# BioinformaticsToolsmith/MeShClust

Hardware: AMD Instinct MI355X
Metric: sequences clustered/sec (+ NW cell-updates/sec) at 1/2/4/8 MI355X (higher is better)
Workload: dtype u8

## Files before the change

meshclust_amd/csrc/gpu/accum_impl.hpp:

```cpp
#pragma once
#include <algorithm>
#include <cstdlib>
#include <cstring>

#include "bvec_core.hpp"
#include "features.hpp"

namespace mcg {

namespace {

constexpr int NT = 512;
constexpr int NW = NT / 64;
constexpr uint32_t NONE = 0xffffffffu;
constexpr uint64_t NONE64 = ~0ull;
constexpr uint32_t RING = 64;
constexpr uint32_t TRACE_STEPS = 4096;
constexpr int TRACE_W = 20;
constexpr uint32_t TRACE2_STEPS = 256;
constexpr int T2W = 6;
constexpr int KINL = 4;
constexpr int REC_HDR = 14;
constexpr uint32_t REC_EXACT = 0x80000000u, REC_THIN = 0x40000000u, REC_KMASK = 0x3fffffffu;
constexpr int PART_G = 8;
// ... 53 lines not shown
  int etake;
  int xfast;
  int thin;
  int rpoll;
  int rpoll_gap;
  uint32_t rec_g;
  uint64_t *klog;
  uint32_t *go;
  uint64_t *partials;
  uint32_t *fpos;
  uint64_t fcap;
  int res;
  uint4 *cc;
  uint4 *srows;
  uint32_t dres;
  uint32_t mrow;
  uint32_t *mem_pos;
  uint64_t *mkeys;
  uint32_t *cl_centre;
  uint64_t *cl_off;
  uint64_t *out;
  uint64_t budget;
  int prof;
  uint64_t *trace;
  int trace_all;
  uint64_t *trace2;
  uint32_t W, rank;
  uint64_t *mbox;
  uint64_t slot_g;
};

__device__ __forceinline__ uint64_t now() { return __builtin_amdgcn_s_memrealtime(); }

typedef unsigned int u32x4_t __attribute__((ext_vector_type(4)));
__device__ __forceinline__ uint4 ld_nt16(const uint4 *p) {
  const u32x4_t v = __builtin_nontemporal_load(reinterpret_cast<const u32x4_t *>(p));
  return make_uint4(v.x, v.y, v.z, v.w);
}

#define MC_LDS __attribute__((address_space(3)))
#define MC_GLB __attribute__((address_space(1)))
__device__ __forceinline__ uint32_t lds_u32(const uint32_t *p) { return *(const MC_LDS uint32_t *)p; }
__device__ __forceinline__ uint64_t lds_u64(const uint64_t *p) { return *(const MC_LDS uint64_t *)p; }
__device__ __forceinline__ uint4 lds_u4(const uint4 *p) {
  const u32x4_t v = *(const MC_LDS u32x4_t *)p;
  return make_uint4(v.x, v.y, v.z, v.w);
}
__device__ __forceinline__ void glb_st16(MC_GLB u32x4_t *p, const uint4 &v) { *p = (u32x4_t){v.x, v.y, v.z, v.w}; }
__device__ __forceinline__ void lds_st16(MC_LDS u32x4_t *p, const uint4 &v) { *p = (u32x4_t){v.x, v.y, v.z, v.w}; }
__device__ __forceinline__ uint4 lds_ld16(const MC_LDS u32x4_t *p) {
  const u32x4_t v = *p;
  return make_uint4(v.x, v.y, v.z, v.w);
}
__device__ __forceinline__ WinTab lds_wt(const WinTab *p) {
  static_assert(sizeof(WinTab) == 40, "WinTab is read as five 8-byte words");
  const MC_LDS uint64_t *q = (const MC_LDS uint64_t *)p;
  uint64_t w[5];
#pragma unroll
  for (int i = 0; i < 5; i++) w[i] = q[i];
  WinTab r;
  __builtin_memcpy(&r, w, sizeof(WinTab));
  return r;
}

__device__ __forceinline__ void trace_mark(const AccArgs &A, uint32_t step, int slot, uint64_t t) {
  if (!A.trace || !A.trace_all || step >= TRACE_STEPS) return;
// ... 508 lines not shown
            uint4 v[NC];
#pragma unroll
            for (int k = 0; k < NC; k++)
              v[k] = from_hs ? A.hs[(uint64_t)k * A.npad + pos] : ld_nt16(creg + (uint64_t)k * NT + t);
            const PInfo pi{A.mag_s[pos], A.sumsq_s[pos], A.len_s[pos]};
            Acc<T> acc;
            double cv;
#pragma unroll
            for (int k = 0; k < NC; k++) acc.add(v[k], clds[k]);
            if (classify_cand<T>(acc, pi, pc, A.B, C, &cv)) {
              lal[(uint64_t)li * NT + sl] = 0;
              flag_pos(pos);
            }
            if (cv > -1.0 && better(cv, pos, best_v, best_p)) {
              best_v = cv;
              best_p = pos;
            }
          }
        }
      }
    } else
    for (uint64_t ch = c0 + mine; ch <= c1; ch += GW) {
      const uint64_t li = dgw.div((uint32_t)ch);
      const uint64_t pos = (ch * A.W + A.rank) * NT + threadIdx.x;
      uint8_t *la = lal + li * NT + threadIdx.x;
      if (!(pos >= P_S && pos <= P_E && *la)) continue;
      nscan++;
      if (trace && threadIdx.x == 0) t_top = now();
      Acc<T> acc;
      double cv;
      if ((int64_t)li < res) {
        const uint4 *rr = lrow + li * (uint64_t)nch * NT + threadIdx.x;
        if constexpr (NCH > 0) {
          constexpr int HB = NC >= 8 ? 8 : NC;
#pragma unroll
          for (int k0 = 0; k0 < NC; k0 += HB) {
            uint4 rv[HB], cvv[HB];
#pragma unroll
            for (int k = 0; k < HB; k++) {
              rv[k] = rr[(uint64_t)(k0 + k) * NT];
              cvv[k] = clds[k0 + k];
            }
#pragma unroll
            for (int k = 0; k < HB; k++) acc.add(rv[k], cvv[k]);
          }
        } else {
          for (int k = 0; k < nch; k++) acc.add(rr[(uint64_t)k * NT], clds[k]);
        }
        if constexpr (sizeof(T) == 1)
          if (trace && threadIdx.x == 0) {
            acc.fold();
            asm volatile("" ::"v"(acc.sad), "v"(acc.dot));
            t_sad = now();
          }
        int d;
        if (li < 2 && C.layout) {
          const PInfo pi = li == 0 ? rinf0 : rinf1;
          d = classify_std(C, acc.finish(pi.mag, pc.mag), pi, li == 0 ? rterm0 : rterm1, pc, tq, A.B, &cv);
#ifdef MC_EXP_DOUBLE_CLASSIFY
          {
            double cv2;
            PInfo p2 = pi;
            const uint64_t z = (uint64_t)(A.budget >> 62);
            p2.len += z;
            p2.mag += z;
            p2.sumsq += z;
            const int d2 = classify_std(C, acc.finish(p2.mag, pc.mag), p2, pterms(p2.mag, p2.sumsq, A.B), pc, tq, A.B, &cv2);
// ... 276 lines not shown
    const PTerms tq = pterms_mk(pc.mag, pc.sumsq, A.B, A.fc.rB);
    const PSm ps_q = psmall(pc, tq);
    const double kq = (double)((int64_t)pc.mag - (int64_t)A.B * tq.ap);
    {
      const uint32_t kinl0 = kend > (uint32_t)KINL ? kend - KINL : 0;
      const uint64_t t0k = kinl0 > kcur ? now() : 0;
      for (uint32_t e = kcur; e < kend; e++) {
        uint32_t p;
        if (e >= kinl0) {
          p = hdr[4 + KINL - (kend - e)];
        } else {
          uint64_t g = ld64(A.klog + e);
          for (uint32_t it = 1; (uint32_t)(g >> 32) != e + 1; it++) {
            if ((it & 255) == 0 && timed_out(A, t0k)) {
              s_abort = 1;
              break;
            }
            __builtin_amdgcn_s_sleep(1);
            g = ld64(A.klog + e);
          }
          p = (uint32_t)g;
        }
        if (p == pos_t) al_t = false;
      }
      kcur = kend;
    }
    if (trace && t == 0) t_klog = now();
    const bool comp = al_t && pos_t >= P_S && pos_t <= P_E;
    int d_t = 0;
    double cv_t = -1.0;
    if (comp) {
      Acc<T> acc;
      const uint4 *rr = lrow + t;
      constexpr int HB = NC >= 8 ? 8 : NC;
      const SmallK sk = lds_smallk(&s_sk);
      if constexpr (NCH > 0) {
#pragma unroll
        for (int k0 = 0; k0 < NC; k0 += HB) {
          uint4 rv[HB], cvv[HB];
#pragma unroll
          for (int k = 0; k < HB; k++) {
            rv[k] = rr[(uint64_t)(k0 + k) * NT];
            cvv[k] = clds[k0 + k];
          }
#pragma unroll
          for (int k = 0; k < HB; k++) acc.add(rv[k], cvv[k]);
        }
      } else {
        for (int k = 0; k < nch; k++) acc.add(rr[(uint64_t)k * NT], clds[k]);
      }
      bool und = true;
      if constexpr (sizeof(T) == 1) {
        if (small_on && ps_q.ok && ps_t.ok) {
          acc.fold();
          d_t = classify_small(sk, acc.sad, acc.dot, ps_t, ps_q, kq, pt_t.da, tq.da, A.B, &cv_t, &und);
          if (und) {
            double cx;
            d_t = classify_std(C, acc.finish(pi_t.mag, pc.mag), pi_t, pt_t, pc, tq, A.B, &cx);
            und = false;
          }
        }
      }
      if (und)
        d_t = A.fc.on    ? classify_fast(C, A.fc, acc.finish(pi_t.mag, pc.mag), pi_t, pt_t, pc, tq, A.B, &cv_t)
              : C.layout ? classify_std(C, acc.finish(pi_t.mag, pc.mag), pi_t, pt_t, pc, tq, A.B, &cv_t)
                         : classify_cand<T>(acc, pi_t, pc, A.B, C, &cv_t);
    }
// ... 566 lines not shown
          }
          lpos[nxt][r] = lp[e];
        }
        base += tot;
        __syncthreads();
      }
      drain();
      __syncthreads();
      n_ent = base;
      alive = 0;
      for (uint32_t j = 0; j < J; j++)
        if (t + NT * j < n_ent) alive |= 1u << j;
      cur = nxt;
    }
  }
}

template <typename T, int NCH, bool WIDE, int TSZ, bool PROF>
__device__ __forceinline__ void controller(const AccArgs &A, uint4 *dyn) {
  [[maybe_unused]] const bool prof_on = PROF && A.prof;
  [[maybe_unused]] uint64_t *const trace = PROF ? A.trace : nullptr;
  [[maybe_unused]] uint64_t *const trace2 = PROF ? A.trace2 : nullptr;
  __shared__ uint64_t s_red[3 * NW];
  __shared__ double s_bv[NW];
  __shared__ uint64_t s_bp[NW];
  __shared__ uint32_t s_new;
  __shared__ uint32_t s_plist[PLIST];
  __shared__ uint32_t s_pbin[PLIST];
  __shared__ uint64_t s_q[4];
  __shared__ uint32_t s_klast[KINL];
  __shared__ uint32_t s_span_all;
  __shared__ int s_abort;
  __shared__ uint64_t s_sumF;
  __shared__ double s_xv[64];
  __shared__ uint64_t s_xp[64];
  __shared__ uint32_t s_xn[64], s_xs[64], s_xi[64][MBOX_INL];
  constexpr int NC = NCH > 0 ? NCH : 1;
  const uint32_t GW = gridDim.x - 1;
  const int lane = threadIdx.x & 63, wv = wave_id();
  const int nch = NCH > 0 ? NCH : A.nch;
  const int rec_words = (int)A.rec_g;
  uint8_t *Fl = reinterpret_cast<uint8_t *>(dyn);
  uint64_t *msum = reinterpret_cast<uint64_t *>(Fl + (size_t)nch * 16);
  uint32_t *cnt = reinterpret_cast<uint32_t *>(msum + A.B);
  uint32_t *fw = cnt + ((A.nb + 1) & ~1u);
  uint32_t *lo = fw + ((A.nb + 2) & ~1u);
  uint64_t *bnd = reinterpret_cast<uint64_t *>(lo + ((A.nb + 2) & ~1u));
  uint32_t *lbits = reinterpret_cast<uint32_t *>(bnd + A.nb);
  const uint64_t nwords = (A.N + 31) / 32;
  MemberCache mc;
  {
    uint8_t *p = reinterpret_cast<uint8_t *>(lbits + (A.gbits ? 0 : (nwords + 3) / 4 * 4));
    mc.rp = WIDE ? 0 : nch + 1;
    mc.row = reinterpret_cast<uint4 *>(p);
    p += (size_t)A.mrow * mc.rp * 16;
    mc.wt = reinterpret_cast<WinTab *>(p);
    p += (size_t)A.mrow * sizeof(WinTab);
    mc.info = reinterpret_cast<uint64_t *>(p);
    p += (size_t)A.mrow * 24;
    mc.key = reinterpret_cast<uint64_t *>(p);
    p += (size_t)A.mrow * 8;
    mc.pos = reinterpret_cast<uint32_t *>(p);
  }
  for (int i = threadIdx.x; i < nch * 16; i += NT) Fl[i] = 0;
  if (threadIdx.x == 0) {
    s_abort = 0;
    s_new = 0;
  }
  uint64_t lg = 1;
  while (lg * 2 <= A.nb) lg *= 2;
  const __amdgpu_buffer_rsrc_t prs =
      __builtin_amdgcn_make_buffer_rsrc(A.partials, 0, (int)(GW * PART_G * 8), 0x00020000);
  DevBvec bv{A.gbits, (MC_LDS uint32_t *)lbits, A.gbits != nullptr, cnt, fw, lo, bnd, A.len_s, A.nb, lg};
  uint32_t last = NONE;
  uint32_t last_q = 0;
  uint64_t cl_start = 0;
  uint64_t M = 0;
  uint64_t ncl = 0, nsteps = 0, ncand = 0;
  uint32_t step = 0;
  uint64_t err = 0;
  uint32_t kn = 0;
  bool rec_exact = false;
  bool thin_out = false;
  uint32_t npend = 0;
  uint64_t t_wait = 0, t_coll = 0, t_mark = 0;
  const uint64_t clk0 = prof_on ? __builtin_amdgcn_s_memtime() : 0, rt0 = prof_on ? now() : 0;
  uint64_t t_sub[4] = {0, 0, 0, 0};
  uint64_t t_ws[4] = {0, 0, 0, 0};
  uint64_t t_cl[3] = {0, 0, 0};
  uint64_t t_pub[2] = {0, 0};
  uint64_t t_wk[5] = {0, 0, 0, 0, 0};

  constexpr uint32_t BK = 64;
  auto finish_cluster = [&]() {
    if (threadIdx.x == BK) {
      A.cl_centre[ncl] = last;
      A.cl_off[ncl + 1] = cl_start + M;
    }
    ncl++;
    cl_start += M;
    M = 0;
  };
  auto log_kill = [&](uint64_t p) {
    if (threadIdx.x == BK) st64(A.klog + kn, gran(kn + 1, (uint32_t)p));
    if (threadIdx.x == 0) s_klast[kn % KINL] = (uint32_t)p;
  };
  auto new_cluster = [&](uint64_t pos, bool kill = false, bool logged = false) {
    if (A.mrow && !WIDE)
      for (int c = threadIdx.x; c < nch; c += NT) mc.row[c] = A.hr[pos * nch + c];
    for (int b = threadIdx.x; b < A.B; b += NT) msum[b] = reinterpret_cast<const T *>(A.hr + pos * nch)[b];
    if (kill && !logged) log_kill(pos);
    if (threadIdx.x == 0) {
      if (A.mrow) {
// ... 18 lines not shown
    M = 1;
    last_q = 0;
    if (kill && !logged) kn++;
    __syncthreads();
  };
  auto pop = [&]() -> uint64_t {
    const int64_t b = bv.first_nonempty();
    if (b < 0) return NONE64;
    const uint64_t p = bv.select((uint64_t)b, 0);
    if (threadIdx.x == 0) bv.kill_in(p, (uint64_t)b);
    log_kill(p);
    kn++;
    __syncthreads();
    return p;
  };
  auto rec_word = [&](int j, bool have, uint64_t S, uint64_t E) -> uint32_t {
    const bool cached = last_q < A.mrow;
    if (!WIDE && j < 4 * nch) {
      if (last == NONE) return 0;
      const uint4 v = cached ? lds_u4(mc.row + (size_t)last_q * mc.rp + j / 4) : A.hr[(uint64_t)last * nch + j / 4];
      return (j & 3) == 0 ? v.x : (j & 3) == 1 ? v.y : (j & 3) == 2 ? v.z : v.w;
    }
    const int h = j - (WIDE ? 0 : 4 * nch);
    if (h == 0) return have ? last : NONE;
    if (h == 1) return (uint32_t)S;
    if (h == 2) return (uint32_t)E;
    if (h == 3) return kn | (rec_exact ? 0x80000000u : 0u);
    if (h < 4 + KINL) {
      const int64_t e = (int64_t)kn - KINL + (h - 4);
      return e >= 0 ? s_klast[e % KINL] : NONE;
    }
    if (last == NONE) return 0;
    const int f = (h - 4 - KINL) / 2, hi = (h - 4 - KINL) & 1;
    const uint64_t v =
        cached ? lds_u64(mc.info + (size_t)last_q * 3 + f) : (f == 0 ? A.mag_s[last] : f == 1 ? A.sumsq_s[last] : A.len_s[last]);
    return hi ? (uint32_t)(v >> 32) : (uint32_t)v;
  };

  auto rec_word_cached = [&](int j, bool have, uint64_t S, uint64_t E) -> uint32_t {
    const int h = j - 4 * nch;
    const int64_t e = (int64_t)kn - KINL + (h - 4);
    const MC_LDS uint32_t *row = (const MC_LDS uint32_t *)(mc.row + (size_t)last_q * mc.rp);
    const MC_LDS uint32_t *inf = (const MC_LDS uint32_t *)(mc.info + (size_t)last_q * 3);
    const MC_LDS uint32_t *p = h < 0               ? row + j
                               : h < 4 + KINL      ? (const MC_LDS uint32_t *)s_klast + (e >= 0 ? (uint32_t)e % KINL : 0u)
                                                   : inf + (h - 4 - KINL);
    const uint32_t x = *p;
    if (h < 0) return x;
    if (h == 0) return have ? last : NONE;
    if (h == 1) return (uint32_t)S;
    if (h == 2) return (uint32_t)E;
    if (h == 3) return kn | (rec_exact ? 0x80000000u : 0u);
    if (h < 4 + KINL) return e >= 0 ? x : NONE;
    return x;
  };
  constexpr int PW = 4;
  auto rec_read = [&](int j0, uint64_t S, uint64_t E, bool have, uint32_t (&d)[PW]) {
    const bool fastw = !WIDE && last != NONE && last_q < A.mrow;
    if (fastw) {
#pragma unroll
      for (int u = 0; u < PW; u++) {
        const int j = j0 + u * 64 + lane;
        d[u] = j < rec_words ? rec_word_cached(j, have, S, E) : 0u;
      }
    } else {
#pragma unroll
      for (int u = 0; u < PW; u++) {
        const int j = j0 + u * 64 + lane;
// ... 5 lines not shown
    uint64_t *r = A.ring + (uint64_t)(step % RING) * A.rec_g;
#pragma unroll
    for (int u = 0; u < PW; u++) {
      const int j = j0 + u * 64 + lane;
      if (j < rec_words) st64(r + j, gran(step, d[u]));
    }
  };
  auto publish_thin = [&](uint32_t pos) {
    const int h = lane;
    const int64_t e = (int64_t)kn - KINL + (h - 4);
    const uint32_t kx = s_klast[e >= 0 ? (uint32_t)e % KINL : 0u];
    const uint32_t x = h == 0 ? pos : h == 1 ? 0u : h == 2 ? (uint32_t)(A.N - 1) : h == 3 ? (kn | REC_THIN)
                     : h < 4 + KINL ? (e >= 0 ? kx : NONE) : 0u;
    if (4 * nch + h < rec_words) st64(A.ring + (uint64_t)(step % RING) * A.rec_g + 4 * nch + h, gran(step, x));
    if (lane == 0) st32(A.go, step);
  };
  auto publish = [&](uint64_t S, uint64_t E, bool have) {
    for (int j0 = 0; j0 < rec_words; j0 += 64 * PW) {
      uint32_t d[PW];
      rec_read(j0, S, E, have, d);
      rec_store(j0, d);
    }
    if (lane == 0) st32(A.go, step);
  };

  auto take = [&](uint64_t qm, uint32_t p, bool sums, int64_t defer = -1) {
    const uint64_t key = ((uint64_t)step << 32) | p;
    const uint4 *hrow = A.hr + (uint64_t)p * nch;
    const bool cached = qm < A.mrow;
    uint2 w[MINFO_W];
    minfo_issue(A.minfo + p, w);
    if constexpr (!WIDE && NCH > 0) {
      if (cached) {
        uint4 rv[NC];
#pragma unroll
        for (int k = 0; k < NC; k++) rv[k] = hrow[k];
#pragma unroll
        for (int k = 0; k < NC; k++) asm volatile("" : "+v"(rv[k].x), "+v"(rv[k].y), "+v"(rv[k].z), "+v"(rv[k].w));
#pragma unroll
        for (int k = 0; k < NC; k++) mc.row[qm * mc.rp + k] = rv[k];
      }
    } else if (!WIDE && cached) {
      for (int k = 0; k < nch; k++) mc.row[qm * mc.rp + k] = hrow[k];
    }
    const MInfo mi = minfo_take(w);
    st32(A.mem_pos + cl_start + qm, p);
    st64(A.mkeys + cl_start + qm, key);
    if (cached) {
      mc.pos[qm] = p;
      mc.key[qm] = key;
      mc.info[qm * 3 + 0] = mi.mag;
      mc.info[qm * 3 + 1] = mi.sumsq;
      mc.info[qm * 3 + 2] = mi.len;
      mc.wt[qm] = mi.wt;
    }
    if (WIDE ? sums : qm >= A.mrow) {
      constexpr int per = 16 / (int)sizeof(T);
      for (int k = 0; k < nch; k++) {
        const uint4 v = hrow[k];
        const T *pv = reinterpret_cast<const T *>(&v);
#pragma unroll
        for (int e = 0; e < per; e++)
          if (pv[e]) atomicAdd((unsigned long long *)&msum[k * per + e], (unsigned long long)pv[e]);
      }
    }
    if (defer >= 0) s_pbin[defer] = (uint32_t)mi.bin;
    else bv.kill_in(p, mi.bin);
  };

  for (uint64_t i = threadIdx.x; i <= A.nb; i += NT) lo[i] = A.bin_lo[i];
  for (uint64_t i = threadIdx.x; i < A.nb; i += NT) {
    bnd[i] = A.bounds[i];
    cnt[i] = A.bin_lo[i + 1] - A.bin_lo[i];
  }
  __syncthreads();
  for (uint64_t i = threadIdx.x + 1; i <= A.nb; i += NT) {
    uint32_t t = 0;
    for (uint64_t b = i - (i & (~i + 1)); b < i; b++) t += cnt[b];
    fw[i] = t;
  }
  if (!A.gbits)
    for (uint64_t x = threadIdx.x; x < nwords; x += NT) {
      const uint64_t rem = A.N - x * 32;
      lbits[x] = rem >= 32 ? ~0u : ((1u << rem) - 1u);
    }
  if (threadIdx.x == 0) {
    A.cl_off[0] = 0;
    s_span_all = 0;
  }
  __syncthreads();
  {
    const uint64_t p = pop();
    if (p != NONE64) {
      last = (uint32_t)p;
      new_cluster(p);
    }
  }

  for (;;) {
    if (prof_on && threadIdx.x == 0) t_mark = now();
// ... 62 lines not shown
        if (thin_out && wv == 0 && lane < 2) st64(A.ringb + (uint64_t)(step % RING) * 2 + lane, gran(step, (uint32_t)(lane ? E : S)));
        thin_out = false;
        if (prof_on && threadIdx.x == 0) {
          const uint64_t t = now();
          t_ws[1] += t - t_mark;
          t_mark = t;
        }
        have = true;
        break;
      }
      const bool ef = wt.fb < A.nb && cnt[wt.fb] > 0, eb = wt.bb < A.nb && cnt[wt.bb] > 0;
      bool fast = wt.fb < A.nb && wt.bb < A.nb && ((ef && eb) || A.xfast);
      int64_t count = 0;
      if (fast) {
        if (wv < 4) {
          const uint64_t pf = lo[wt.fb] + wt.kf, qb = lo[wt.bb] + wt.kble;
          uint64_t r;
          if (wv == 0) r = ef ? bv.next_alive(pf, lo[wt.fb + 1]) : bv.first_alive_of(bv.first_nonempty());
          else if (wv == 1) r = ef ? bv.prev_alive(lo[wt.fb], pf) : NONE64;
          else if (wv == 2) r = eb ? bv.next_alive(qb, lo[wt.bb + 1]) : bv.first_alive_of(bv.last_nonempty());
          else r = eb ? bv.prev_alive(lo[wt.bb], qb) : NONE64;
          if (lane == 0) s_q[wv] = r;
        }
        __syncthreads();
        const uint64_t q0 = s_q[0], q1 = s_q[1], q2 = s_q[2], q3 = s_q[3];
        __syncthreads();
        fast = (ef || q0 != NONE64) && (eb || q2 != NONE64);
        if (fast) {
          bv_fast_window(q0, q1, q2, q3, lo[wt.bb] + wt.kblt, &S, &E);
          count = (S != NONE64 && E != NONE64 && E >= S) ? 1 : 0;
        }
      }
      if (!fast) {
        bv.h = wt;
        BPos f, b;
        bv_get_range(bv, wt.bl, wt.el, f, b);
        int e = 0;
        count = bv_window(bv, f, b, &S, &E, &e);
        if (e) {
          err = 10 + e;
          if (A.spec && wv == 0 && lane < 2) st64(A.ringb + (uint64_t)(step % RING) * 2 + lane, gran(step, NONE));
          break;
        }
      }
      if (prof_on && threadIdx.x == 0) {
        const uint64_t t = now();
        t_ws[1] += t - t_mark;
        t_mark = t;
        t_wk[fast ? 1 : 2] += t - tk0;
        t_wk[fast ? 3 : 4]++;
      }
      thin_out = false;
      if (count > 0) {
        have = true;
        if (A.spec && wv == 0 && lane < 2) st64(A.ringb + (uint64_t)(step % RING) * 2 + lane, gran(step, (uint32_t)(lane ? E : S)));
        break;
      }
      if (A.spec && wv == 0 && lane < 2) st64(A.ringb + (uint64_t)(step % RING) * 2 + lane, gran(step, NONE));
      const uint64_t p = pop();
      finish_cluster();
      last = p == NONE64 ? NONE : (uint32_t)p;
      if (p != NONE64) new_cluster(p);
    }
    if (have) nsteps++;
    if (!A.spec || !have) {
      step++;
      if (wv == 0) publish(S, E, have);
    }
    if (prof_on && threadIdx.x == 0) {
      const uint64_t t = now();
      t_ws[2] += t - t_mark;
      t_mark = t;
      if (trace && step < TRACE_STEPS) trace[(uint64_t)step * TRACE_W + 0] = t;
    }
    if (!have) break;

    constexpr uint64_t TS = (uint64_t)TSZ;
    uint64_t c0 = 0, c1 = 0;
    const uint32_t nact = rank_tiles(S / TS, E / TS, A.W, A.rank, &c0, &c1)
                              ? (uint32_t)(c1 - c0 + 1 < (uint64_t)GW ? c1 - c0 + 1 : (uint64_t)GW)
                              : 0u;
    uint64_t *mslot = A.mbox ? A.mbox + ((uint64_t)(step & 1) * A.W + A.rank) * A.slot_g : nullptr;
    constexpr uint32_t P0 = 64;
    const uint32_t pt = threadIdx.x - P0;
    double bv_ = -1.0;
    uint64_t bp_ = NONE64;
    uint32_t cnt_w = 0, scan_w = 0;
    if (threadIdx.x >= P0 && pt < nact) {
      const uint32_t wk = Div32(GW).mod((uint32_t)c0 + pt);
      const uint64_t *q = A.partials + (uint64_t)wk * PART_G;
      const uint32_t poff = wk * PART_G * 8;
      const uint64_t t0 = now();
      uint64_t g8[PART_G];
      for (uint32_t it = 1;; it++) {
        bool ok = true;
        if (A.poll1) {
          ok = (uint32_t)(ld64(q + 4 + INL) >> 32) == step;
          if (ok) {
#pragma unroll
            for (int j = 0; j < 5 + INL; j++) {
              g8[j] = ld64(q + j);
              ok &= (uint32_t)(g8[j] >> 32) == step;
            }
          }
        } else {
#pragma unroll
          for (int j = 0; j < PART_G / 2; j++) {
            const u32x4_t v = __builtin_amdgcn_raw_buffer_load_b128(prs, (int)(poff + 16 * j), 0, 16);
            g8[2 * j] = ((uint64_t)v.y << 32) | v.x;
            g8[2 * j + 1] = ((uint64_t)v.w << 32) | v.z;
          }
#pragma unroll
          for (int j = 0; j < 5 + INL; j++) ok &= (uint32_t)(g8[j] >> 32) == step;
        }
        if (ok) break;
// ... 68 lines not shown
    {
      const uint32_t fl = lane < NW ? (uint32_t)s_red[lane] : 0u, sc = lane < NW ? (uint32_t)s_red[NW + lane] : 0u;
      double v = lane < NW ? s_bv[lane] : -1.0;
      uint64_t p = lane < NW ? s_bp[lane] : NONE64;
      nflag = wave_sum32(fl);
      nsc = wave_sum32(sc);
      const double m = wave_ext_f64_all<true>(v);
      const uint64_t hit = __ballot(p != NONE64 && v == m);
      if (__popcll(hit) > 1) {
        wave_best_all(v, p, better);
        best_val = v;
        best_pos = p;
      } else if (hit) {
        const int L = __builtin_ctzll(hit);
        best_val = __builtin_bit_cast(double, readlane64(__builtin_bit_cast(uint64_t, v), L));
        best_pos = readlane64(p, L);
      } else {
        best_val = -1.0;
        best_pos = NONE64;
      }
    }
    if (mslot) {
      if (threadIdx.x >= BK && threadIdx.x < BK + MBOX_HDR) {
        const uint64_t vb = (uint64_t)__double_as_longlong(best_val);
        const int j = threadIdx.x - BK;
        const uint32_t data = j == 0   ? (uint32_t)(vb >> 32)
                              : j == 1 ? (uint32_t)vb
                              : j == 2 ? (best_pos == NONE64 ? NONE : (uint32_t)best_pos)
                              : j == 3 ? (uint32_t)nflag
                              : j == 4 ? (uint32_t)nsc
                                       : NONE;
        if (j < 5 || (uint64_t)(j - 5) >= nflag) st64x(mslot + j, gran(step, data));
      }
      uint64_t *mbase = A.mbox + (uint64_t)(step & 1) * A.W * A.slot_g;
      if (threadIdx.x < A.W) {
        const uint64_t *h = mbase + (uint64_t)threadIdx.x * A.slot_g;
        const uint64_t t0 = now();
        uint64_t g[MBOX_HDR];
        for (uint32_t it = 1;; it++) {
          bool ok = true;
#pragma unroll
          for (int j = 0; j < MBOX_HDR; j++) {
            g[j] = ld64x(h + j);
            ok &= (uint32_t)(g[j] >> 32) == step;
          }
          if (ok) break;
          if ((it & 63) == 0 && timed_out(A, t0)) {
            s_abort = 1;
            break;
          }
          __builtin_amdgcn_s_sleep(1);
        }
        s_xv[threadIdx.x] = __longlong_as_double((long long)((g[0] << 32) | (g[1] & 0xffffffffull)));
        s_xp[threadIdx.x] = (uint32_t)g[2] == NONE ? NONE64 : (uint64_t)(uint32_t)g[2];
        s_xn[threadIdx.x] = (uint32_t)g[3];
        s_xs[threadIdx.x] = (uint32_t)g[4];
#pragma unroll
        for (int j = 0; j < MBOX_INL; j++) s_xi[threadIdx.x][j] = (uint32_t)g[5 + j];
      }
      __syncthreads();
      if (s_abort) {
        if (threadIdx.x == 0) atomicMax((unsigned long long *)&A.out[3], 99ull);
        return;
      }
      nflag = 0;
      nsc = 0;
      best_val = -1.0;
      best_pos = NONE64;
      for (uint32_t r = 0; r < A.W; r++) {
        nflag += s_xn[r];
        nsc += s_xs[r];
        if (s_xp[r] != NONE64 && better(s_xv[r], s_xp[r], best_val, best_pos)) {
          best_val = s_xv[r];
          best_pos = s_xp[r];
        }
      }
      for (uint64_t i = threadIdx.x; i < nflag; i += NT) {
        uint32_t r = 0;
        uint64_t j = i;
        while (j >= s_xn[r]) j -= s_xn[r++];
        const uint64_t *e = mbase + (uint64_t)r * A.slot_g + MBOX_HDR - MBOX_INL + j;
        const uint64_t t0 = now();
        uint64_t g = j < (uint64_t)MBOX_INL ? gran(step, s_xi[r][j]) : ld64x(e);
        for (uint32_t it = 1; (uint32_t)(g >> 32) != step; it++) {
          if ((it & 63) == 0 && timed_out(A, t0)) {
            s_abort = 1;
            break;
          }
          __builtin_amdgcn_s_sleep(1);
          g = ld64x(e);
        }
        if (i < PLIST) {
          s_plist[i] = (uint32_t)g;
        } else {
          take(M + i, (uint32_t)g, true);
          drain();
        }
      }
      __syncthreads();
      if (s_abort) {
        if (threadIdx.x == 0) atomicMax((unsigned long long *)&A.out[3], 99ull);
        return;
      }
    }
    ncand += nsc;
    uint64_t tq = 0;
    if (prof_on && threadIdx.x == 0) {
      tq = now();
      t_sub[0] += tq - t_mark;
    }
    if (nflag > 0) {
      if (!A.etake || mslot)
        for (uint64_t i = (threadIdx.x + NT - 64) % NT; i < nflag && i < PLIST; i += NT)
          take(M + i, s_plist[i], false, (int64_t)i);
      npend = nflag < PLIST ? (uint32_t)nflag : PLIST;
      if (M + nflag > A.mrow) drain();
      __syncthreads();
      if (prof_on && threadIdx.x == 0) t_ws[3] += now() - tq;
      const uint64_t q0 = M, q1 = M + nflag < A.mrow ? M + nflag : (uint64_t)A.mrow;
      const uint32_t nlist = nflag < PLIST ? (uint32_t)nflag : PLIST;
      M += nflag;
      if constexpr (WIDE) {
        constexpr int per = 16 / (int)sizeof(T);
        const int nsl = nch >= NT ? 1 : NT / nch;
        for (int t = threadIdx.x; t < nch * nsl; t += NT) {
          const int c = t % nch, sl = t / nch;
          uint32_t sum[per];
#pragma unroll
          for (int e = 0; e < per; e++) sum[e] = 0;
          uint32_t i = (uint32_t)sl;
          for (; i + 7u * (uint32_t)nsl < nlist; i += 8u * (uint32_t)nsl) {
            uint4 v[8];
#pragma unroll
            for (int u = 0; u < 8; u++) v[u] = A.hr[(uint64_t)s_plist[i + (uint32_t)u * (uint32_t)nsl] * nch + c];
#pragma unroll
            for (int u = 0; u < 8; u++) {
              const T *pv = reinterpret_cast<const T *>(&v[u]);
#pragma unroll
              for (int e = 0; e < per; e++) sum[e] += pv[e];
            }
          }
          for (; i < nlist; i += (uint32_t)nsl) {
            const uint4 v = A.hr[(uint64_t)s_plist[i] * nch + c];
            const T *pv = reinterpret_cast<const T *>(&v);
#pragma unroll
            for (int e = 0; e < per; e++) sum[e] += pv[e];
          }
#pragma unroll
          for (int e = 0; e < per; e++)
            if (sum[e] && c * per + e < A.B) atomicAdd((unsigned long long *)&msum[c * per + e], (unsigned long long)sum[e]);
        }
      } else {
        constexpr int per = 4 / (int)sizeof(T);
        const int wpr = (A.B + per - 1) / per;
        const int nsl = wpr >= NT ? 1 : NT / wpr;
        for (int t = threadIdx.x; t < wpr * nsl; t += NT) {
          const int wd = t % wpr, sl = t / wpr;
          uint32_t sum[per];
#pragma unroll
          for (int e = 0; e < per; e++) sum[e] = 0;
          for (uint64_t q = q0 + (uint64_t)sl; q < q1; q += (uint64_t)nsl) {
            const uint32_t x = reinterpret_cast<const uint32_t *>(mc.row + q * mc.rp)[wd];
#pragma unroll
            for (int e = 0; e < per; e++) sum[e] += sizeof(T) == 1 ? (x >> (8 * e)) & 0xffu : (x >> (16 * e)) & 0xffffu;
          }
#pragma unroll
          for (int e = 0; e < per; e++)
            if (sum[e] && wd * per + e < A.B) atomicAdd((unsigned long long *)&msum[wd * per + e], (unsigned long long)sum[e]);
        }
      }
      __syncthreads();
      if (prof_on && threadIdx.x == 0) {
        const uint64_t t = now();
        t_sub[1] += t - tq;
        tq = t;
      }
      uint64_t part = 0;
      for (int b = threadIdx.x; b < A.B; b += NT) {
        const uint64_t sb = msum[b];
        const uint64_t F = (sb >> 32) == 0 ? (uint64_t)((uint32_t)sb / (uint32_t)M) : sb / M;
        reinterpret_cast<T *>(Fl)[b] = (T)F;
        part += F;
      }
      part = wave_sum64_all(part);
      if (lane == 0 && part) atomicAdd((unsigned long long *)&s_sumF, (unsigned long long)part);
      __syncthreads();
      if (prof_on && threadIdx.x == 0) {
        const uint64_t t = now();
        t_sub[2] += t - tq;
        tq = t;
      }
      const uint64_t sumF = s_sumF;
      const uint4 *F4 = reinterpret_cast<const uint4 *>(Fl);
      double bd = __builtin_inf();
      uint64_t bk = NONE64, bq = 0;
      if constexpr (WIDE) {
        auto member_row = [&](uint64_t q) -> const uint4 * {
          const uint32_t r = q < A.mrow ? lds_u32(mc.pos + q) : ld32(A.mem_pos + cl_start + q);
          return A.hr + (uint64_t)r * nch;
        };
        auto score = [&](uint64_t q, Acc<T> &acc) {
          const uint64_t mp = q < A.mrow ? lds_u64(mc.info + q * 3) : A.mag_s[ld32(A.mem_pos + cl_start + q)];
          const uint64_t key = q < A.mrow ? lds_u64(mc.key + q) : ld64(A.mkeys + cl_start + q);
          const PS s = acc.finish(mp, sumF);
          const double frac = (double)(2 * s.smin) / (double)(mp + sumF);
          const double d = __builtin_fma(-frac, frac, 1.0) * 10000.0;
          if (d < bd || (d == bd && key < bk)) {
            bd = d;
            bk = key;
            bq = q;
          }
        };
        if (nch <= 256) {
          auto load = [&](uint64_t q, uint4 (&v)[4]) {
            const uint4 *row = member_row(q < M ? q : (uint64_t)wv);
#pragma unroll
            for (int u = 0; u < 4; u++) {
              const int c = lane + 64 * u;
              v[u] = row[c < nch ? c : nch - 1];
            }
          };
          auto reduce = [&](uint64_t q, const uint4 (&v)[4]) {
            Acc<T> acc;
#pragma unroll
            for (int u = 0; u < 4; u++) {
// ... 5 lines not shown
          };
          uint4 va[4], vb[4];
          uint64_t q = wv;
          if (q < M) {
            load(q, va);
            for (;;) {
              load(q + NW, vb);
              reduce(q, va);
              q += NW;
              if (q >= M) break;
              load(q + NW, va);
              reduce(q, vb);
              q += NW;
              if (q >= M) break;
            }
          }
        } else {
          for (uint64_t q = wv; q < M; q += NW) {
            const uint4 *row = member_row(q);
            Acc<T> acc;
            int c = lane;
            for (; c + 192 < nch; c += 256) {
              const uint4 v0 = row[c], v1 = row[c + 64], v2 = row[c + 128], v3 = row[c + 192];
              acc.add_sad(v0, F4[c]);
              acc.add_sad(v1, F4[c + 64]);
              acc.add_sad(v2, F4[c + 128]);
              acc.add_sad(v3, F4[c + 192]);
            }
            for (; c < nch; c += 64) acc.add_sad(row[c], F4[c]);
            acc.wave_reduce();
            score(q, acc);
          }
        }
      } else if (NCH > 0 && NC % 4 == 0 && sizeof(T) == 1 && (A.dbg & 2)) {
        constexpr int CPL = NC >= 4 ? NC / 4 : 1;
        const int sub = threadIdx.x & 3;
        for (uint64_t q = threadIdx.x >> 2; q < M; q += NT / 4) {
          uint32_t s4[CPL];
          if (q < A.mrow) {
            const uint4 *row = mc.row + q * mc.rp + sub * CPL;
            uint4 rv[CPL], fv[CPL];
#pragma unroll
            for (int k = 0; k < CPL; k++) {
              rv[k] = row[k];
              fv[k] = F4[sub * CPL + k];
            }
#pragma unroll
            for (int k = 0; k < CPL; k++) {
              s4[k] = __builtin_amdgcn_sad_u8(rv[k].x, fv[k].x, 0u);
              s4[k] = __builtin_amdgcn_sad_u8(rv[k].y, fv[k].y, s4[k]);
              s4[k] = __builtin_amdgcn_sad_u8(rv[k].z, fv[k].z, s4[k]);
              s4[k] = __builtin_amdgcn_sad_u8(rv[k].w, fv[k].w, s4[k]);
            }
          } else {
            const uint64_t r = ld32(A.mem_pos + cl_start + q);
#pragma unroll
            for (int k = 0; k < CPL; k++) {
              const uint4 a = A.hr[r * nch + sub * CPL + k], f = F4[sub * CPL + k];
              s4[k] = __builtin_amdgcn_sad_u8(a.x, f.x, 0u);
              s4[k] = __builtin_amdgcn_sad_u8(a.y, f.y, s4[k]);
              s4[k] = __builtin_amdgcn_sad_u8(a.z, f.z, s4[k]);
              s4[k] = __builtin_amdgcn_sad_u8(a.w, f.w, s4[k]);
            }
          }
          uint32_t sad = 0;
#pragma unroll
          for (int k = 0; k < CPL; k++) sad += s4[k];
          sad += dpp_mv<0xB1>(0u, sad);
          sad += dpp_mv<0x4E>(0u, sad);
          if (sub == 0) {
            const uint64_t mp = q < A.mrow ? lds_u64(mc.info + q * 3) : A.mag_s[ld32(A.mem_pos + cl_start + q)];
            const uint64_t key = q < A.mrow ? lds_u64(mc.key + q) : ld64(A.mkeys + cl_start + q);
            const uint64_t smin = (mp + sumF - sad) >> 1;
            const double frac = (double)(2 * smin) / (double)(mp + sumF);
            const double d = __builtin_fma(-frac, frac, 1.0) * 10000.0;
            if (d < bd || (d == bd && key < bk)) {
              bd = d;
              bk = key;
              bq = q;
            }
          }
        }
      } else
      for (uint64_t q = threadIdx.x; q < M; q += NT) {
        Acc<T> acc;
        uint64_t mp, key;
        if (q < A.mrow) {
          const uint4 *row = mc.row + q * mc.rp;
          if constexpr (NCH > 0) {
            constexpr int HB = NC >= 8 ? 8 : NC;
#pragma unroll
            for (int k0 = 0; k0 < NC; k0 += HB) {
              uint4 rv[HB], fv[HB];
#pragma unroll
              for (int k = 0; k < HB; k++) {
                rv[k] = row[k0 + k];
                fv[k] = F4[k0 + k];
              }
#pragma unroll
              for (int k = 0; k < HB; k++) acc.add_sad(rv[k], fv[k]);
            }
          } else {
            for (int k = 0; k < nch; k++) acc.add_sad(row[k], F4[k]);
          }
          mp = mc.info[q * 3];
          key = mc.key[q];
        } else {
          const uint64_t r = ld32(A.mem_pos + cl_start + q);
          for (int k = 0; k < nch; k++) acc.add_sad(A.hr[r * nch + k], F4[k]);
          mp = A.mag_s[r];
          key = ld64(A.mkeys + cl_start + q);
        }
        const PS s = acc.finish(mp, sumF);
        const double frac = (double)(2 * s.smin) / (double)(mp + sumF);
        const double d = __builtin_fma(-frac, frac, 1.0) * 10000.0;
        if (d < bd || (d == bd && key < bk)) {
          bd = d;
          bk = key;
          bq = q;
        }
      }
      uint64_t tc0 = 0;
      if (prof_on && threadIdx.x == 0) {
        tc0 = now();
        t_cl[0] += tc0 - tq;
      }
      {
        const double md = wave_ext_f64_all<false>(bd);
        uint64_t hit = __ballot(bk != NONE64 && bd == md);
        double rd = md;
        uint64_t rk = NONE64;
        if (__popcll(hit) > 1) {
          rd = bd;
          rk = bk;
          wave_best_all(rd, rk, [](double a, uint64_t ka, double b, uint64_t kb) { return a < b || (a == b && ka < kb); });
          hit = __ballot(bd == rd && bk == rk);
        }
        const int L = hit ? __builtin_ctzll(hit) : 0;
        if (hit) rk = readlane64(bk, L);
        bq = readlane64(bq, L);
        bd = hit ? rd : __builtin_inf();
        bk = rk;
      }
// ... 33 lines not shown
      if (win < A.mrow) last = lds_u32(mc.pos + win);
      else last = ld32(A.mem_pos + cl_start + win);
      if (threadIdx.x == 0) s_new = 0;
      if (prof_on && threadIdx.x == 0) {
        const uint64_t t = now();
        t_sub[3] += t - tq;
        t_cl[2] += t - tc1;
      }
    } else if (best_pos != NONE64) {
      finish_cluster();
      last = (uint32_t)best_pos;
      thin_out = A.thin && s_span_all;
      if (thin_out) {
        log_kill(best_pos);
        kn++;
        step++;
        if (wv == 0) publish_thin((uint32_t)best_pos);
      }
      new_cluster(best_pos, true, thin_out);
    } else {
      const uint64_t p = pop();
      finish_cluster();
      last = p == NONE64 ? NONE : (uint32_t)p;
      if (p != NONE64) new_cluster(p);
    }
    if (prof_on && threadIdx.x == 0) {
      const uint64_t t = now();
      t_coll += t - t_mark;
      if (trace && step < TRACE_STEPS) trace[(uint64_t)step * TRACE_W + 8] = t;
    }
  }
  if (threadIdx.x == 0) {
    A.out[0] = ncl;
    A.out[1] = nsteps;
    A.out[2] = ncand;
    if (err) atomicMax((unsigned long long *)&A.out[3], (unsigned long long)err);
    A.out[4] = cl_start;
    A.out[5] = t_ws[0] + t_ws[1] + t_ws[2];
    A.out[6] = t_wait;
    A.out[7] = t_coll;
    for (int i = 0; i < 4; i++) A.out[8 + i] = t_sub[i];
    for (int i = 0; i < 4; i++) A.out[12 + i] = t_ws[i];
    for (int i = 0; i < 3; i++) A.out[18 + i] = t_cl[i];
    for (int i = 0; i < 2; i++) A.out[21 + i] = t_pub[i];
    for (int i = 0; i < 5; i++) A.out[23 + i] = t_wk[i];
    if (prof_on) {
      A.out[16] = __builtin_amdgcn_s_memtime() - clk0;
      A.out[17] = now() - rt0;
    }
  }
}

template <typename T, int NCH, bool WIDE = false, bool CPT = false, bool DENSE = false, bool DSTREAM = false, bool PROF = false>
__global__ __launch_bounds__(NT) void accum_kernel(AccArgs A, DevClassifier C) {
  extern __shared__ __attribute__((aligned(16))) uint4 dyn[];
  constexpr int TSZ = (DENSE || DSTREAM) ? DT : WIDE ? NW : NT;
  if (blockIdx.x == 0) controller<T, NCH, WIDE, TSZ, PROF>(A, dyn);
  else if constexpr (DENSE) worker_dense<T, NCH, PROF>(A, C, dyn);
  else if constexpr (DSTREAM) worker_dstream<T, NCH>(A, C, dyn);
  else worker<T, NCH, WIDE, CPT, PROF>(A, C, dyn);
}

}

}
```

Measured before the change: 2.805 million.

## Cut controller register pressure and parallelise member row intake and centroid sums

The controller kernel stops keeping rarely used pointers live: they are reloaded from the kernarg segment, step counters move into shared memory, and unroll widths drop from 8 to 4. New member rows are copied into the LDS cache cooperatively, 16 lanes per row. The non-wide centroid sum now uses slice-parallel packed byte adds with DPP reductions, folding the per-bin division into the same pass and recomputing sumF per wave. The quad-lane scoring path is enabled for small clusters by default. Together these aim to cut VGPR spills and serial per-thread work on the critical single-block path, at the risk of extra kernarg loads and subtle correctness issues in the reworked reductions.

```diff
diff --git a/meshclust_amd/csrc/gpu/accum_impl.hpp b/meshclust_amd/csrc/gpu/accum_impl.hpp
--- a/meshclust_amd/csrc/gpu/accum_impl.hpp
+++ b/meshclust_amd/csrc/gpu/accum_impl.hpp
@@ -109,6 +109,12 @@
 
 __device__ __forceinline__ uint64_t now() { return __builtin_amdgcn_s_memrealtime(); }
 
+#define MC_KARG __attribute__((address_space(4)))
+__device__ __forceinline__ const MC_KARG AccArgs *args_again() {
+  const MC_KARG AccArgs *p = (const MC_KARG AccArgs *)__builtin_amdgcn_kernarg_segment_ptr();
+  return p;
+}
+
 typedef unsigned int u32x4_t __attribute__((ext_vector_type(4)));
 __device__ __forceinline__ uint4 ld_nt16(const uint4 *p) {
   const u32x4_t v = __builtin_nontemporal_load(reinterpret_cast<const u32x4_t *>(p));
@@ -683,7 +689,7 @@
       if ((int64_t)li < res) {
         const uint4 *rr = lrow + li * (uint64_t)nch * NT + threadIdx.x;
         if constexpr (NCH > 0) {
-          constexpr int HB = NC >= 8 ? 8 : NC;
+          constexpr int HB = NC >= 4 ? 4 : NC;
 #pragma unroll
           for (int k0 = 0; k0 < NC; k0 += HB) {
             uint4 rv[HB], cvv[HB];
@@ -1026,7 +1032,7 @@
     if (comp) {
       Acc<T> acc;
       const uint4 *rr = lrow + t;
-      constexpr int HB = NC >= 8 ? 8 : NC;
+      constexpr int HB = NC >= 4 ? 4 : NC;
       const SmallK sk = lds_smallk(&s_sk);
       if constexpr (NCH > 0) {
 #pragma unroll
@@ -1659,6 +1665,7 @@
   __shared__ uint32_t s_span_all;
   __shared__ int s_abort;
   __shared__ uint64_t s_sumF;
+  __shared__ uint64_t s_stat[2];
   __shared__ double s_xv[64];
   __shared__ uint64_t s_xp[64];
   __shared__ uint32_t s_xn[64], s_xs[64], s_xi[64][MBOX_INL];
@@ -1693,19 +1700,21 @@
   if (threadIdx.x == 0) {
     s_abort = 0;
     s_new = 0;
+    s_stat[0] = s_stat[1] = 0;
   }
   uint64_t lg = 1;
   while (lg * 2 <= A.nb) lg *= 2;
   const __amdgpu_buffer_rsrc_t prs =
       __builtin_amdgcn_make_buffer_rsrc(A.partials, 0, (int)(GW * PART_G * 8), 0x00020000);
   DevBvec bv{A.gbits, (MC_LDS uint32_t *)lbits, A.gbits != nullptr, cnt, fw, lo, bnd, A.len_s, A.nb, lg};
+  const bool ranks = A.mbox != nullptr;
   uint32_t last = NONE;
   uint32_t last_q = 0;
   uint64_t cl_start = 0;
   uint64_t M = 0;
-  uint64_t ncl = 0, nsteps = 0, ncand = 0;
+  uint64_t ncl = 0;
   uint32_t step = 0;
-  uint64_t err = 0;
+  uint32_t err = 0;
   uint32_t kn = 0;
   bool rec_exact = false;
   bool thin_out = false;
@@ -1790,8 +1799,13 @@
     }
     if (last == NONE) return 0;
     const int f = (h - 4 - KINL) / 2, hi = (h - 4 - KINL) & 1;
-    const uint64_t v =
-        cached ? lds_u64(mc.info + (size_t)last_q * 3 + f) : (f == 0 ? A.mag_s[last] : f == 1 ? A.sumsq_s[last] : A.len_s[last]);
+    uint64_t v;
+    if (cached) {
+      v = lds_u64(mc.info + (size_t)last_q * 3 + f);
+    } else {
+      const MC_KARG AccArgs *R = args_again();
+      v = f == 0 ? R->mag_s[last] : f == 1 ? R->sumsq_s[last] : R->len_s[last];
+    }
     return hi ? (uint32_t)(v >> 32) : (uint32_t)v;
   };
 
@@ -1863,13 +1877,17 @@
     minfo_issue(A.minfo + p, w);
     if constexpr (!WIDE && NCH > 0) {
       if (cached) {
-        uint4 rv[NC];
-#pragma unroll
-        for (int k = 0; k < NC; k++) rv[k] = hrow[k];
-#pragma unroll
-        for (int k = 0; k < NC; k++) asm volatile("" : "+v"(rv[k].x), "+v"(rv[k].y), "+v"(rv[k].z), "+v"(rv[k].w));
-#pragma unroll
-        for (int k = 0; k < NC; k++) mc.row[qm * mc.rp + k] = rv[k];
+        constexpr int QB = NC % 4 == 0 ? 4 : 1;
+#pragma unroll 1
+        for (int k0 = 0; k0 < NC; k0 += QB) {
+          uint4 rv[QB];
+#pragma unroll
+          for (int k = 0; k < QB; k++) rv[k] = hrow[k0 + k];
+#pragma unroll
+          for (int k = 0; k < QB; k++) asm volatile("" : "+v"(rv[k].x), "+v"(rv[k].y), "+v"(rv[k].z), "+v"(rv[k].w));
+#pragma unroll
+          for (int k = 0; k < QB; k++) mc.row[qm * mc.rp + k0 + k] = rv[k];
+        }
       }
     } else if (!WIDE && cached) {
       for (int k = 0; k < nch; k++) mc.row[qm * mc.rp + k] = hrow[k];
@@ -1897,6 +1915,62 @@
     }
     if (defer >= 0) s_pbin[defer] = (uint32_t)mi.bin;
     else bv.kill_in(p, mi.bin);
+  };
+  auto take_rows = [&](uint32_t n) {
+    constexpr int TL = 16, TG = NT / TL, TU = 4;
+    constexpr int KPL = NCH > 0 ? (NC + TL - 1) / TL : (WIDE_NCH + TL - 1) / TL;
+    static_assert(MINFO_W + 2 <= TL, "a lane per MInfo word, position and key");
+    const int c = threadIdx.x & (TL - 1), g = threadIdx.x / TL;
+    for (uint32_t i0 = 0; i0 < n; i0 += TG * TU) {
+      uint4 rv[TU][KPL];
+      uint2 mw[TU];
+      uint32_t pp[TU];
+#pragma unroll
+      for (int u = 0; u < TU; u++) {
+        const uint32_t i = i0 + (uint32_t)(u * TG + g);
+        pp[u] = s_plist[i < n ? i : 0u];
+        const uint4 *hrow = A.hr + (uint64_t)pp[u] * nch;
+#pragma unroll
+        for (int k = 0; k < KPL; k++) {
+          const int ch = k * TL + c;
+          rv[u][k] = hrow[ch < nch ? ch : nch - 1];
+        }
+        mw[u] = reinterpret_cast<const uint2 *>(A.minfo + pp[u])[c < MINFO_W ? c : 0];
+      }
+#pragma unroll
+      for (int u = 0; u < TU; u++) {
+#pragma unroll
+        for (int k = 0; k < KPL; k++) asm volatile("" : "+v"(rv[u][k].x), "+v"(rv[u][k].y), "+v"(rv[u][k].z), "+v"(rv[u][k].w));
+        asm volatile("" : "+v"(mw[u].x), "+v"(mw[u].y));
+      }
+#pragma unroll
+      for (int u = 0; u < TU; u++) {
+        const uint32_t i = i0 + (uint32_t)(u * TG + g);
+        if (i < n) {
+          const uint64_t qm = M + i;
+#pragma unroll
+          for (int k = 0; k < KPL; k++) {
+            const int ch = k * TL + c;
+            if (ch < nch) lds_st16((MC_LDS u32x4_t *)(mc.row + qm * mc.rp + ch), rv[u][k]);
+          }
+          const uint64_t w = ((uint64_t)mw[u].y << 32) | mw[u].x;
+          if (c < 3) *(MC_LDS uint64_t *)(mc.info + qm * 3 + c) = w;
+          else if (c == 3) s_pbin[i] = (uint32_t)w;
+          else if (c < MINFO_W) *((MC_LDS uint64_t *)(mc.wt + qm) + (c - 4)) = w;
+          else if (c == MINFO_W) *(MC_LDS uint32_t *)(mc.pos + qm) = pp[u];
+          else if (c == MINFO_W + 1) *(MC_LDS uint64_t *)(mc.key + qm) = ((uint64_t)step << 32) | pp[u];
+        }
+      }
+    }
+  };
+  auto list_rows = [&](uint64_t q0, uint32_t n) {
+    uint32_t i1 = (threadIdx.x + NT - 64) % NT;
+    asm volatile("" : "+v"(i1));
+    for (uint32_t i = i1; i < n; i += NT) {
+      const uint32_t p = s_plist[i];
+      st32(A.mem_pos + cl_start + q0 + i, p);
+      st64(A.mkeys + cl_start + q0 + i, ((uint64_t)step << 32) | p);
+    }
   };
 
   for (uint64_t i = threadIdx.x; i <= A.nb; i += NT) lo[i] = A.bin_lo[i];
@@ -2025,11 +2099,12 @@
         }
       }
       if (!fast) {
-        bv.h = wt;
+        DevBvec bh = bv;
+        bh.h = wt;
         BPos f, b;
-        bv_get_range(bv, wt.bl, wt.el, f, b);
+        bv_get_range(bh, wt.bl, wt.el, f, b);
         int e = 0;
-        count = bv_window(bv, f, b, &S, &E, &e);
+        count = bv_window(bh, f, b, &S, &E, &e);
         if (e) {
           err = 10 + e;
           if (A.spec && wv == 0 && lane < 2) st64(A.ringb + (uint64_t)(step % RING) * 2 + lane, gran(step, NONE));
@@ -2055,7 +2130,7 @@
       last = p == NONE64 ? NONE : (uint32_t)p;
       if (p != NONE64) new_cluster(p);
     }
-    if (have) nsteps++;
+    if (have && threadIdx.x == 0) s_stat[0]++;
     if (!A.spec || !have) {
       step++;
       if (wv == 0) publish(S, E, have);
@@ -2073,7 +2148,11 @@
     const uint32_t nact = rank_tiles(S / TS, E / TS, A.W, A.rank, &c0, &c1)
                               ? (uint32_t)(c1 - c0 + 1 < (uint64_t)GW ? c1 - c0 + 1 : (uint64_t)GW)
                               : 0u;
-    uint64_t *mslot = A.mbox ? A.mbox + ((uint64_t)(step & 1) * A.W + A.rank) * A.slot_g : nullptr;
+    uint64_t *mslot = nullptr;
+    if (ranks) {
+      const MC_KARG AccArgs *R = args_again();
+      mslot = R->mbox + ((uint64_t)(step & 1) * A.W + A.rank) * R->slot_g;
+    }
     constexpr uint32_t P0 = 64;
     const uint32_t pt = threadIdx.x - P0;
     double bv_ = -1.0;
@@ -2208,9 +2287,10 @@
                                        : NONE;
         if (j < 5 || (uint64_t)(j - 5) >= nflag) st64x(mslot + j, gran(step, data));
       }
-      uint64_t *mbase = A.mbox + (uint64_t)(step & 1) * A.W * A.slot_g;
+      const uint64_t slot_g = args_again()->slot_g;
+      uint64_t *mbase = args_again()->mbox + (uint64_t)(step & 1) * A.W * slot_g;
       if (threadIdx.x < A.W) {
-        const uint64_t *h = mbase + (uint64_t)threadIdx.x * A.slot_g;
+        const uint64_t *h = mbase + (uint64_t)threadIdx.x * slot_g;
         const uint64_t t0 = now();
         uint64_t g[MBOX_HDR];
         for (uint32_t it = 1;; it++) {
@@ -2255,7 +2335,7 @@
         uint32_t r = 0;
         uint64_t j = i;
         while (j >= s_xn[r]) j -= s_xn[r++];
-        const uint64_t *e = mbase + (uint64_t)r * A.slot_g + MBOX_HDR - MBOX_INL + j;
+        const uint64_t *e = mbase + (uint64_t)r * slot_g + MBOX_HDR - MBOX_INL + j;
         const uint64_t t0 = now();
         uint64_t g = j < (uint64_t)MBOX_INL ? gran(step, s_xi[r][j]) : ld64x(e);
         for (uint32_t it = 1; (uint32_t)(g >> 32) != step; it++) {
@@ -2279,22 +2359,31 @@
         return;
       }
     }
-    ncand += nsc;
+    if (threadIdx.x == 0) s_stat[1] += nsc;
     uint64_t tq = 0;
     if (prof_on && threadIdx.x == 0) {
       tq = now();
       t_sub[0] += tq - t_mark;
     }
     if (nflag > 0) {
-      if (!A.etake || mslot)
-        for (uint64_t i = (threadIdx.x + NT - 64) % NT; i < nflag && i < PLIST; i += NT)
+      uint32_t nrow = 0;
+      if (!A.etake || mslot) {
+        const uint32_t nl = nflag < PLIST ? (uint32_t)nflag : PLIST;
+        if constexpr (!WIDE) {
+          if (NCH > 0 || nch <= WIDE_NCH)
+            nrow = M >= A.mrow ? 0u : (uint64_t)nl < A.mrow - M ? nl : (uint32_t)(A.mrow - M);
+          if (nrow) take_rows(nrow);
+        }
+        for (uint64_t i = nrow + (threadIdx.x + NT - 64) % NT; i < nl; i += NT)
           take(M + i, s_plist[i], false, (int64_t)i);
+      }
       npend = nflag < PLIST ? (uint32_t)nflag : PLIST;
       if (M + nflag > A.mrow) drain();
       __syncthreads();
       if (prof_on && threadIdx.x == 0) t_ws[3] += now() - tq;
       const uint64_t q0 = M, q1 = M + nflag < A.mrow ? M + nflag : (uint64_t)A.mrow;
       const uint32_t nlist = nflag < PLIST ? (uint32_t)nflag : PLIST;
+      if (nrow) list_rows(M, nrow);
       M += nflag;
       if constexpr (WIDE) {
         constexpr int per = 16 / (int)sizeof(T);
@@ -2326,47 +2415,98 @@
           for (int e = 0; e < per; e++)
             if (sum[e] && c * per + e < A.B) atomicAdd((unsigned long long *)&msum[c * per + e], (unsigned long long)sum[e]);
         }
+        __syncthreads();
+        if (prof_on && threadIdx.x == 0) {
+          const uint64_t t = now();
+          t_sub[1] += t - tq;
+          tq = t;
+        }
+        uint64_t part = 0;
+        for (int b = threadIdx.x; b < A.B; b += NT) {
+          const uint64_t sb = msum[b];
+          const uint64_t F = (sb >> 32) == 0 ? (uint64_t)((uint32_t)sb / (uint32_t)M) : sb / M;
+          reinterpret_cast<T *>(Fl)[b] = (T)F;
+          part += F;
+        }
+        part = wave_sum64_all(part);
+        if (lane == 0 && part) atomicAdd((unsigned long long *)&s_sumF, (unsigned long long)part);
       } else {
         constexpr int per = 4 / (int)sizeof(T);
+        constexpr int NSL = 8;
         const int wpr = (A.B + per - 1) / per;
-        const int nsl = wpr >= NT ? 1 : NT / wpr;
-        for (int t = threadIdx.x; t < wpr * nsl; t += NT) {
-          const int wd = t % wpr, sl = t / wpr;
+        for (int t0 = 0; t0 < wpr * NSL; t0 += NT) {
+          const int t = t0 + threadIdx.x;
+          const int sl = t & (NSL - 1), wd = t / NSL;
           uint32_t sum[per];
 #pragma unroll
           for (int e = 0; e < per; e++) sum[e] = 0;
-          for (uint64_t q = q0 + (uint64_t)sl; q < q1; q += (uint64_t)nsl) {
-            const uint32_t x = reinterpret_cast<const uint32_t *>(mc.row + q * mc.rp)[wd];
-#pragma unroll
-            for (int e = 0; e < per; e++) sum[e] += sizeof(T) == 1 ? (x >> (8 * e)) & 0xffu : (x >> (16 * e)) & 0xffffu;
-          }
-#pragma unroll
-          for (int e = 0; e < per; e++)
-            if (sum[e] && wd * per + e < A.B) atomicAdd((unsigned long long *)&msum[wd * per + e], (unsigned long long)sum[e]);
-        }
-      }
-      __syncthreads();
-      if (prof_on && threadIdx.x == 0) {
-        const uint64_t t = now();
-        t_sub[1] += t - tq;
-        tq = t;
-      }
-      uint64_t part = 0;
-      for (int b = threadIdx.x; b < A.B; b += NT) {
-        const uint64_t sb = msum[b];
-        const uint64_t F = (sb >> 32) == 0 ? (uint64_t)((uint32_t)sb / (uint32_t)M) : sb / M;
-        reinterpret_cast<T *>(Fl)[b] = (T)F;
-        part += F;
-      }
-      part = wave_sum64_all(part);
-      if (lane == 0 && part) atomicAdd((unsigned long long *)&s_sumF, (unsigned long long)part);
+          if (wd < wpr) {
+            const MC_LDS uint32_t *col = (const MC_LDS uint32_t *)mc.row + wd;
+            const uint32_t rw = (uint32_t)mc.rp * 4u, qe = (uint32_t)q1;
+            if constexpr (sizeof(T) == 1) {
+              static_assert(PLIST / NSL * 255u < 65536u, "a slice's byte sums fit 16 bits");
+              uint32_t ev = 0, od = 0;
+#pragma unroll 4
+              for (uint32_t q = (uint32_t)q0 + (uint32_t)sl; q < qe; q += NSL) {
+                const uint32_t x = col[q * rw];
+                ev += x & 0x00ff00ffu;
+                od += (x >> 8) & 0x00ff00ffu;
+              }
+              sum[0] = ev & 0xffffu;
+              sum[1] = od & 0xffffu;
+              sum[2] = ev >> 16;
+              sum[3] = od >> 16;
+            } else {
+#pragma unroll 4
+              for (uint32_t q = (uint32_t)q0 + (uint32_t)sl; q < qe; q += NSL) {
+                const uint32_t x = col[q * rw];
+#pragma unroll
+                for (int e = 0; e < per; e++) sum[e] += (x >> (16 * e)) & 0xffffu;
+              }
+            }
+          }
+#pragma unroll
+          for (int e = 0; e < per; e++) {
+            sum[e] += dpp_mv<0xB1>(0u, sum[e]);
+            sum[e] += dpp_mv<0x4E>(0u, sum[e]);
+            sum[e] += dpp_mv<0x141>(0u, sum[e]);
+          }
+          uint32_t mine = sum[0];
+#pragma unroll
+          for (int e = 1; e < per; e++) mine = sl == e ? sum[e] : mine;
+          const int b = wd * per + sl;
+          if (sl < per && b < A.B) {
+            const uint64_t sb = lds_u64(msum + b) + mine;
+            *(MC_LDS uint64_t *)(msum + b) = sb;
+            const uint64_t F = (sb >> 32) == 0 ? (uint64_t)((uint32_t)sb / (uint32_t)M) : sb / M;
+            *((MC_LDS T *)Fl + b) = (T)F;
+          }
+        }
+        if (prof_on && threadIdx.x == 0) {
+          const uint64_t t = now();
+          t_sub[1] += t - tq;
+          tq = t;
+        }
+      }
       __syncthreads();
       if (prof_on && threadIdx.x == 0) {
         const uint64_t t = now();
         t_sub[2] += t - tq;
         tq = t;
       }
-      const uint64_t sumF = s_sumF;
+      uint64_t sumF;
+      if constexpr (WIDE) {
+        sumF = s_sumF;
+      } else {
+        constexpr int per = 4 / (int)sizeof(T);
+        uint32_t fs = 0;
+        for (int wd = lane; wd < nch * 4; wd += 64) {
+          const uint32_t x = *((const MC_LDS uint32_t *)Fl + wd);
+#pragma unroll
+          for (int e = 0; e < per; e++) fs += sizeof(T) == 1 ? (x >> (8 * e)) & 0xffu : (x >> (16 * e)) & 0xffffu;
+        }
+        sumF = wave_sum32(fs);
+      }
       const uint4 *F4 = reinterpret_cast<const uint4 *>(Fl);
       double bd = __builtin_inf();
       uint64_t bk = NONE64, bq = 0;
@@ -2438,7 +2578,7 @@
             score(q, acc);
           }
         }
-      } else if (NCH > 0 && NC % 4 == 0 && sizeof(T) == 1 && (A.dbg & 2)) {
+      } else if (NCH > 0 && NC % 4 == 0 && sizeof(T) == 1 && (M <= NT / 4 || (A.dbg & 2))) {
         constexpr int CPL = NC >= 4 ? NC / 4 : 1;
         const int sub = threadIdx.x & 3;
         for (uint64_t q = threadIdx.x >> 2; q < M; q += NT / 4) {
@@ -2475,7 +2615,7 @@
           sad += dpp_mv<0xB1>(0u, sad);
           sad += dpp_mv<0x4E>(0u, sad);
           if (sub == 0) {
-            const uint64_t mp = q < A.mrow ? lds_u64(mc.info + q * 3) : A.mag_s[ld32(A.mem_pos + cl_start + q)];
+            const uint64_t mp = q < A.mrow ? lds_u64(mc.info + q * 3) : args_again()->mag_s[ld32(A.mem_pos + cl_start + q)];
             const uint64_t key = q < A.mrow ? lds_u64(mc.key + q) : ld64(A.mkeys + cl_start + q);
             const uint64_t smin = (mp + sumF - sad) >> 1;
             const double frac = (double)(2 * smin) / (double)(mp + sumF);
@@ -2494,7 +2634,7 @@
         if (q < A.mrow) {
           const uint4 *row = mc.row + q * mc.rp;
           if constexpr (NCH > 0) {
-            constexpr int HB = NC >= 8 ? 8 : NC;
+            constexpr int HB = NC >= 4 ? 4 : NC;
 #pragma unroll
             for (int k0 = 0; k0 < NC; k0 += HB) {
               uint4 rv[HB], fv[HB];
@@ -2514,7 +2654,7 @@
         } else {
           const uint64_t r = ld32(A.mem_pos + cl_start + q);
           for (int k = 0; k < nch; k++) acc.add_sad(A.hr[r * nch + k], F4[k]);
-          mp = A.mag_s[r];
+          mp = args_again()->mag_s[r];
           key = ld64(A.mkeys + cl_start + q);
         }
         const PS s = acc.finish(mp, sumF);
@@ -2614,8 +2754,8 @@
   }
   if (threadIdx.x == 0) {
     A.out[0] = ncl;
-    A.out[1] = nsteps;
-    A.out[2] = ncand;
+    A.out[1] = s_stat[0];
+    A.out[2] = s_stat[1];
     if (err) atomicMax((unsigned long long *)&A.out[3], (unsigned long long)err);
     A.out[4] = cl_start;
     A.out[5] = t_ws[0] + t_ws[1] + t_ws[2];
```

Measured after the change: 2.718 million. 3.1% lower.
